# ska-telescope/ska-sdp-screen-fitting

Hardware: AMD Instinct MI355X
Metric: screen-slots/sec (ant×time×freq) + FITS-cube wall-clock, KL 256² screen (higher is better)
Workload: dtype f64

## Files before the change

include/screenfit.h:

```cpp
#ifndef SCREENFIT_H
#define SCREENFIT_H

#include <stddef.h>
#include <stdint.h>

#ifdef __cplusplus
extern "C" {
#endif

#define SF_OK 0
#define SF_EINVAL (-22)
#define SF_ENOMEM (-12)
#define SF_EIO (-5)
#define SF_ENODEV (-19)

#define SF_MAX_DIR 60
#define SF_MAX_FIT_DIR 128
#define SF_MAX_EVAL_DIR 128

#define SF_SCREEN_PHASE 0
#define SF_SCREEN_TEC 1
#define SF_SCREEN_AMPLITUDE 2

#define SF_EVAL_NAN_SCRUB 1u
// ... 21 lines not shown
int sf_synchronize(sf_ctx* ctx);
int sf_stream_create(sf_ctx* ctx, const int* reserve_cus, int n_reserve,
                     void** hip_stream);
int sf_stream_destroy(sf_ctx* ctx, void* hip_stream);
int sf_device_cus(sf_ctx* ctx, int* n_cu);
#define SF_OPT_FIT_GENERAL 1
#define SF_OPT_EVAL_KERNEL 2
#define SF_OPT_EVAL_MAX_BLOCKS 3
#define SF_OPT_FIT_PACK 4
#define SF_OPT_EVAL_KS_PAD 5
#define SF_OPT_EVAL_SLEEP 6
#define SF_OPT_EVAL_XCD_MAP 7
#define SF_OPT_EVAL_GROUPS 8
#define SF_OPT_EVAL_BANDS 9
#define SF_OPT_FIT_LEAN 10
#define SF_OPT_TESS_SLOTS 11
#define SF_OPT_TESS_WAVES 12
#define SF_OPT_TESS_TILE 13
#define SF_OPT_TESS_BOX 14
#define SF_OPT_EVAL_INT 15
#define SF_OPT_EVAL_WG_WAVES 16
#define SF_OPT_FIT_EIG_WAVES 17
#define SF_OPT_FIT_SUBSET_DELETION 18
#define SF_EVAL_KERNEL_AUTO 0
#define SF_EVAL_KERNEL_TILE 1
#define SF_EVAL_KERNEL_LDS4 2
#define SF_EVAL_KERNEL_LDS8 3
#define SF_EVAL_KERNEL_LDS16 4
#define SF_EVAL_KERNEL_LDS8H 5
#define SF_EVAL_KERNEL_LDS16H 6
#define SF_EVAL_KERNEL_TILE3 7
#define SF_EVAL_KERNEL_SHB 8
#define SF_EVAL_KERNEL_WIDE 9
int sf_get_eval_kernel(sf_ctx* ctx, int gain, unsigned flags, int* kernel);
#define SF_EVAL_CONTRACTION_F64 0
#define SF_EVAL_CONTRACTION_I8_DIGITS 1
int sf_get_eval_contraction(sf_ctx* ctx, int gain, unsigned flags, int* contraction);
int sf_set_option(sf_ctx* ctx, int option, int value);
int sf_alloc(sf_ctx* ctx, size_t bytes, void** dev_ptr);
int sf_free(sf_ctx* ctx, void* dev_ptr);
int sf_copy_h2d(sf_ctx* ctx, void* dst_dev, const void* src_host, size_t bytes);
int sf_copy_d2h(sf_ctx* ctx, void* dst_host, const void* src_dev, size_t bytes);

int sf_set_basis(sf_ctx* ctx, const double* pp_host, int D, double r0,
                 double beta);
int sf_set_basis_wide(sf_ctx* ctx, const double* pp_host, int D, double r0,
                      double beta);
int sf_get_basis(sf_ctx* ctx, double* c_host, double* pinv_c_host,
                 double* u_host, double* eig_host);

int sf_set_piercepoints(sf_ctx* ctx, const double* pp_host, int D, double r0,
                        double beta);

int sf_kl_fit(sf_ctx* ctx, const double* phase, const float* weight, int T,
              int F, int A, const int* station_order_host,
              const sf_fit_params* params, double* coef, double* resid,
              float* w_out, int32_t* order_out);

int sf_get_fit_stats(sf_ctx* ctx, int* n_masks, int* n_general);

int sf_get_fit_pool(sf_ctx* ctx, uint64_t* masks_host, double* entries_host,
                    int max_masks, int* n_masks);

int sf_set_grid(sf_ctx* ctx, const double* x_host, int nx,
                const double* y_host, int ny);

int sf_kl_eval(sf_ctx* ctx, const double* coef, int64_t S, float* out,
               int64_t ring_slots, unsigned flags);

int sf_kl_eval_gain(sf_ctx* ctx, const double* coef_phase,
                    const double* coef_xx, const double* coef_yy, int64_t S,
                    float* out, int64_t ring_slots, unsigned flags);
int sf_kl_eval_sums(sf_ctx* ctx, const double* coef_phase,
                    const double* coef_xx, const double* coef_yy, int64_t S,
                    float* out, int64_t ring, unsigned flags,
                    uint32_t* slot_sums);

int sf_kl_eval_values(sf_ctx* ctx, const double* coef, int64_t S, float* out,
                      int64_t ring_slots, unsigned flags);

#define SF_MAX_POINTS 4096
int sf_set_points(sf_ctx* ctx, const double* xy_host, int P);
// ... 17 lines not shown
```

ska-sdp-screen-fitting_amd/csrc/capi.hip:

```cpp
#include <hip/hip_runtime.h>

#include <cmath>
#include <cstring>
#include <string>
#include <vector>

#include "sf_internal.h"

namespace sf {
static thread_local std::string g_last_error;
void set_error(const std::string& msg) { g_last_error = msg; }
}

using sf::set_error;

namespace {

int check_device(int device) {
  int n = 0;
  hipError_t e = hipGetDeviceCount(&n);
  if (e != hipSuccess || n == 0) {
    set_error("no HIP device available");
    return SF_ENODEV;
  }
// ... 73 lines not shown
  hipFree(ctx->d_c);
  hipFree(ctx->d_pinv);
  hipFree(ctx->d_u);
  hipFree(ctx->d_eig);
  hipFree(ctx->d_wide_ws);
  hipFree(ctx->d_wide_w);
  hipFree(ctx->d_wide_o);
  hipFree(ctx->d_cfrag);
  hipFree(ctx->d_pxy);
  hipFree(ctx->d_pfrag);
  hipFree(ctx->d_cdig);
  hipFree(ctx->d_kdig);
  hipFree(ctx->d_kflag);
  if (ctx->kdig_read) (void)hipEventDestroy(ctx->kdig_read);
  hipFree(ctx->d_skip);
  hipFree(ctx->d_st_order);
  hipFree(ctx->d_keys);
  hipFree(ctx->d_ids);
  hipFree(ctx->d_pool_mask);
  hipFree(ctx->d_pool);
  hipFree(ctx->d_pool_status);
  hipFree(ctx->d_pos);
  hipFree(ctx->d_sigma);
  hipFree(ctx->d_class);
  hipFree(ctx->d_counters);
  hipFree(ctx->d_scratch);
  hipFree(ctx->d_wscratch);
  hipFree(ctx->d_oscratch);
  hipFree(ctx->d_gw);
  hipFree(ctx->d_smooth);
  hipFree(ctx->d_tess_tab);
  hipFree(ctx->d_trash);
  delete ctx;
  return SF_OK;
}

int sf_set_stream(sf_ctx* ctx, void* stream) {
  SF_REQUIRE(ctx, SF_EINVAL, "sf_set_stream: NULL context");
  ctx->stream = reinterpret_cast<hipStream_t>(stream);
  return SF_OK;
}

int sf_device_cus(sf_ctx* ctx, int* n_cu) {
  SF_REQUIRE(ctx && n_cu, SF_EINVAL, "sf_device_cus: NULL argument");
  SF_HIP(hipDeviceGetAttribute(n_cu, hipDeviceAttributeMultiprocessorCount,
                               ctx->device));
// ... 28 lines not shown
int sf_stream_destroy(sf_ctx* ctx, void* stream) {
  SF_REQUIRE(ctx && stream, SF_EINVAL, "sf_stream_destroy: bad argument");
  SF_HIP(hipSetDevice(ctx->device));
  SF_HIP(hipStreamDestroy(reinterpret_cast<hipStream_t>(stream)));
  return SF_OK;
}

int sf_set_option(sf_ctx* ctx, int option, int value) {
  SF_REQUIRE(ctx, SF_EINVAL, "sf_set_option: NULL context");
  switch (option) {
    case SF_OPT_FIT_GENERAL:
      ctx->force_general = value != 0;
      return SF_OK;
    case SF_OPT_EVAL_KERNEL:
      SF_REQUIRE(value >= SF_EVAL_KERNEL_AUTO && value <= SF_EVAL_KERNEL_WIDE,
                 SF_EINVAL, "sf_set_option: unknown evaluation kernel");
      ctx->eval_kernel = value;
      return SF_OK;
    case SF_OPT_FIT_PACK:
      ctx->fit_pack = value != 0;
      return SF_OK;
    case SF_OPT_FIT_LEAN:
      ctx->fit_lean = value != 0;
      return SF_OK;
    case SF_OPT_EVAL_KS_PAD:
      SF_REQUIRE(value >= 0 && value <= 3, SF_EINVAL,
                 "sf_set_option: k-step padding must be 0..3");
      ctx->eval_ks_pad = value;
      return SF_OK;
    case SF_OPT_EVAL_SLEEP:
      SF_REQUIRE(value >= 0 && value <= 1000, SF_EINVAL,
                 "sf_set_option: eval sleep must be 0..1000");
      ctx->eval_sleep = value;
      return SF_OK;
    case SF_OPT_EVAL_XCD_MAP:
      SF_REQUIRE(value >= -1 && value <= 1, SF_EINVAL,
                 "sf_set_option: XCD map must be -1, 0 or 1");
      ctx->eval_xcd_map = value;
      return SF_OK;
    case SF_OPT_EVAL_GROUPS:
      SF_REQUIRE(value >= 0 && value <= 256 && (value & (value - 1)) == 0,
                 SF_EINVAL, "sf_set_option: groups must be 0 or a power of two <= 256");
      ctx->eval_groups = value;
      return SF_OK;
    case SF_OPT_EVAL_BANDS:
      SF_REQUIRE(value >= 0 && value <= 128 && (value & (value - 1)) == 0,
// ... 251 lines not shown
  }
  if (ctx->st_order_cap < (size_t)A) {
    SF_TRY(dev_alloc(&ctx->d_st_order, (size_t)A));
    ctx->st_order_cap = (size_t)A;
  }
  SF_HIP(hipMemcpyAsync(ctx->d_st_order, st_order, sizeof(int) * A,
                        hipMemcpyHostToDevice, ctx->stream));
  return sf::launch_fit(ctx, phase, weight, T, F, A, p, coef, resid, w_out,
                        order_out);
}

int sf_get_fit_stats(sf_ctx* ctx, int* n_masks, int* n_general) {
  SF_REQUIRE(ctx, SF_EINVAL, "sf_get_fit_stats: NULL context");
  int c[4] = {0, 0, 0, 0};
  SF_HIP(hipSetDevice(ctx->device));
  SF_HIP(hipStreamSynchronize(ctx->stream));
  if (ctx->d_counters)
    SF_HIP(hipMemcpy(c, ctx->d_counters, sizeof(c), hipMemcpyDeviceToHost));
  if (n_masks) *n_masks = c[0];
  if (n_general) *n_general = c[2];
  return SF_OK;
}

int sf_get_fit_pool(sf_ctx* ctx, uint64_t* masks_host, double* entries_host,
                    int max_masks, int* n_masks) {
  SF_REQUIRE(ctx && n_masks && max_masks >= 0, SF_EINVAL, "sf_get_fit_pool: bad argument");
  SF_REQUIRE(max_masks == 0 || (masks_host && entries_host), SF_EINVAL,
             "sf_get_fit_pool: NULL output");
  SF_REQUIRE(!ctx->wide, SF_EINVAL,
             "sf_get_fit_pool: no mask pool above SF_MAX_DIR directions "
             "(sf_set_basis_wide: every flagged slot decomposes its own subset)");
  SF_HIP(hipSetDevice(ctx->device));
  SF_HIP(hipStreamSynchronize(ctx->stream));
  int c0 = 0;
  if (ctx->d_counters)
    SF_HIP(hipMemcpy(&c0, ctx->d_counters, sizeof(int), hipMemcpyDeviceToHost));
  const int n = ctx->pool_D == ctx->D && (size_t)c0 <= ctx->pool_cap ? c0 : 0;
  *n_masks = n;
  const int k = n < max_masks ? n : max_masks;
  if (k > 0) {
    const size_t entry = (size_t)ctx->D * ctx->D + ctx->D;
    SF_HIP(hipMemcpy(masks_host, ctx->d_pool_mask, k * sizeof(uint64_t),
                     hipMemcpyDeviceToHost));
    SF_HIP(hipMemcpy(entries_host, ctx->d_pool, k * entry * sizeof(double),
                     hipMemcpyDeviceToHost));
  }
// ... 289 lines not shown
```

ska-sdp-screen-fitting_amd/csrc/kl_fit_fast.hip:

```cpp
#include <hip/hip_runtime.h>

#include <algorithm>
#include <cmath>
#include <cstdlib>

#include "sf_internal.h"
#include "sf_wave.h"

namespace sf {

constexpr double kAtol = 1e-3;
constexpr size_t kLdsBytes = 160 * 1024;
constexpr double kTinyW = 1e-3 * 1.001;
constexpr unsigned long long kEmptyKey = 0ull;

__host__ __device__ inline int ldo(int n) { return n | 1; }

__device__ __forceinline__ unsigned long long mix64(unsigned long long x) {
  x ^= x >> 30;
  x *= 0xbf58476d1ce4e5b9ull;
  x ^= x >> 27;
  x *= 0x94d049bb133111ebull;
  x ^= x >> 31;
  return x;
}

__device__ int table_insert(unsigned long long* keys, int cap,
                            unsigned long long key) {
  int h = (int)(mix64(key) & (unsigned long long)(cap - 1));
  for (int probe = 0; probe < cap; ++probe) {
    unsigned long long prev = keys[h];
    if (prev == kEmptyKey) prev = atomicCAS(keys + h, kEmptyKey, key);
    if (prev == kEmptyKey || prev == key) return h;
    h = (h + 1) & (cap - 1);
  }
  return -3;
}
// ... 476 lines not shown
  return (size_t)((c_global ? 1 : 2) * D * ldo(D) + 64) * sizeof(double);
}
__host__ __device__ inline size_t fast_wave_bytes(int D, bool slow, bool lean = false) {
  if (lean) return (size_t)6 * 64 * sizeof(double);
  return (size_t)((slow ? 3 : 2) * D * ldo(D) + 64 + 6 * 64) * sizeof(double) +
         (slow ? 64 * sizeof(double2) + 96 * sizeof(int2) : 0);
}

struct Basis {
  int n;
  bool full;
  int ld;
  const double* U;
  const double* lam;
};

__device__ __noinline__ void nl_sincos(double x, double* s, double* c) { sincos(x, s, c); }
__device__ __noinline__ double nl_atan2(double y, double x) { return atan2(y, x); }
__device__ __noinline__ double nl_log10(double x) { return log10(x); }
__device__ __noinline__ double nl_pow(double x, double y) { return pow(x, y); }
__device__ __noinline__ double nl_log(double x) { return log(x); }
__device__ __noinline__ double nl_fmod(double x, double y) { return fmod(x, y); }

template <bool NI>
struct FitMath {
  static __device__ __forceinline__ void sin_cos(double x, double* s, double* c) {
    if constexpr (NI) nl_sincos(x, s, c); else sincos(x, s, c);
  }
  static __device__ __forceinline__ double arctan2(double y, double x) {
    if constexpr (NI) return nl_atan2(y, x); else return atan2(y, x);
  }
  static __device__ __forceinline__ double lg10(double x) {
    if constexpr (NI) return nl_log10(x); else return log10(x);
  }
  static __device__ __forceinline__ double power(double x, double y) {
    if constexpr (NI) return nl_pow(x, y); else return pow(x, y);
  }
  static __device__ __forceinline__ double ln(double x) {
    if constexpr (NI) return nl_log(x); else return log(x);
  }
  static __device__ __forceinline__ double mod(double x, double y) {
    if constexpr (NI) return nl_fmod(x, y); else return fmod(x, y);
  }
};

template <bool NI = false>
// ... 185 lines not shown
    v0[l] = fabs(lm) > kAtol ? sh / lm : 0.0;
  }
  lds_sync();
  double wa = 0.0;
  if (l < D)
#pragma unroll kMatVecUnroll
    for (int r = 0; r < D; ++r) wa += L.U[l * ld + r] * v0[r];
  lds_sync();
  white_d = wa;
  resid_d = phi_d - model_value<NI>(screen_type, sall);
}

template <bool NI = false>
__device__ __forceinline__ double screen_diff(int screen_type, double val,
                                              double resid) {
  if (screen_type == SF_SCREEN_AMPLITUDE)
    return FitMath<NI>::lg10(val) - FitMath<NI>::lg10(fabs(val - resid));
  return resid;
}

#ifndef SF_FIT_MINW
#define SF_FIT_MINW 4
#endif
template <bool SLOW, int SPW, bool LEAN>
__global__ __launch_bounds__(256, SLOW ? 1 : SF_FIT_MINW) void kl_fit_pass_kernel(
    int it, int niter, int64_t S, int F, int A, int D,
    const double* __restrict__ phase, const double* __restrict__ refph,
    int ref_sub, const double* __restrict__ g_u, const double* __restrict__ g_c,
    const double* __restrict__ g_eig, const int* __restrict__ st_order,
    const uint8_t* __restrict__ cls, int* __restrict__ pos,
    const int* __restrict__ ids, unsigned long long* __restrict__ keys, int cap,
    const double* __restrict__ pool, int pool_cap, int* __restrict__ counters,
    int screen_type, double nsigma, int adjust_order, double* __restrict__ coef,
    double* __restrict__ resid, float* __restrict__ w_out,
    int32_t* __restrict__ order_out) {
#pragma clang fp contract(off)
  extern __shared__ double smem[];
  const int ld = ldo(D);
  using G = Group<SPW>;
  using M = FitMath<!SLOW>;
  constexpr bool NI = !SLOW;
  constexpr bool CG = SPW == 1;
  const int nwaves = blockDim.x / 64;
  const int nslots = nwaves * SPW;
  const int wv = (threadIdx.x / 64) * SPW + G::index();
  const int d = G::lane();
  double* sU = smem;
  double* sC = CG ? nullptr : sU + D * ld;
  double* sl = sU + (CG ? 1 : 2) * D * ld;
  for (int e = threadIdx.x; e < D * D; e += blockDim.x) {
    const int r = e / D, c = e % D;
    sU[r * ld + c] = g_u[e];
    if (!CG) sC[r * ld + c] = g_c[e];
  }
  for (int e = threadIdx.x; e < 64; e += blockDim.x) sl[e] = e < D ? g_eig[e] : 0.0;
  __syncthreads();
  FastLds L;
  L.U = sU;
  L.C = CG ? g_c : sC;
  L.cld = CG ? D : ld;
  L.lam = sl;
  double* wb = sl + 64 + (size_t)wv * (fast_wave_bytes(D, SLOW, LEAN) / sizeof(double));
  if (LEAN) {
    L.Vs = L.G = L.M = L.lams = nullptr;
    L.vec = wb;
    L.cs = nullptr;
    L.pr = nullptr;
  } else {
    L.Vs = wb;
    L.G = wb + D * ld;
    L.M = L.G + D * ld;
    L.lams = (SLOW ? L.M + D * ld : L.G + D * ld);
    L.vec = L.lams + 64;
    L.cs = reinterpret_cast<double2*>(L.vec + 6 * 64);
    L.pr = reinterpret_cast<int2*>(L.cs + 64);
  }
  const uint8_t want = SLOW ? 2 : 0;

  for (int64_t s = (int64_t)blockIdx.x * nslots + wv; s < S;
       s += (int64_t)gridDim.x * nslots) {
    if (SLOW && cls[s] != want) continue;
    const uint8_t cl = SLOW ? want : cls[s];
    const int a = (int)(s % A);
    const int p0 = pos[s];
    const int64_t base = s * D;
    double phi_d = 0.0, w_d = 0.0, white_d = 0.0, resid_d = 0.0;
    if (d < D) {
      phi_d = phase_ref(phase, refph, ref_sub, s, a, A, D, d);
      w_d = (double)w_out[base + d];
      white_d = it == 0 ? 0.0 : coef[base + d];
      resid_d = it == 0 ? 0.0 : resid[base + d];
    }
    double order = (double)order_out[s];
    const double station_order = (double)st_order[a];
    if (cl != want) continue;
    int id = -1;
    if (p0 >= 0) {
      id = ids[p0];
      if (id < 0 || id >= pool_cap) {
        if (d == 0) atomicOr(counters + 3, 1);
        continue;
      }
    } else if (p0 == -3) {
      if (d == 0) atomicOr(counters + 3, 2);
      continue;
// ... 20 lines not shown
          if (d < n_unfl) L.Vs[r * ld + d] = e[r * D + d];
        if (d < n_unfl) L.lams[d] = e[D * D + d];
        lds_sync();
        B.U = L.Vs;
        B.lam = L.lams;
      }
    }
    double phi_p = 0.0, w_p = 0.0;
    {
      double* v4 = L.vec + 256;
      double* v5 = L.vec + 320;
      if (unfl) {
        const int p = G::rank(um);
        v4[p] = phi_d;
        v5[p] = w_d;
      }
      lds_sync();
      if (d < n_unfl) {
        phi_p = v4[d];
        w_p = v5[d];
      }
      lds_sync();
    }
    const double wmax = G::max(unfl ? w_d : -INFINITY);
    const double wmin = -G::max(unfl ? -w_d : -INFINITY);
    const bool uniform = (wmax == wmin);
    if (LEAN && n_unfl > 0 && !uniform) {
      if (d == 0) atomicOr(counters + 3, 4);
      continue;
    }

    if (n_unfl > 0) {
      if (order > n_unfl - 1) order = n_unfl - 1;
      if (it == 0) {
        fit_once<SLOW, SPW, LEAN>(L, B, D, ld, (int)order, screen_type, uniform, wmin,
                       phi_p, w_p, phi_d, w_d, white_d, resid_d);
      } else if (adjust_order) {
        bool hit_upper = false, hit_lower = false, hit_upper2 = false,
             hit_lower2 = false;
        double sign = 1.0, prev_redchi2 = 0.0;
        for (int oi = 0; oi < 4; ++oi) {
          if (oi > 0)
            fit_once<SLOW, SPW, LEAN>(L, B, D, ld, (int)order, screen_type, uniform, wmin,
                           phi_p, w_p, phi_d, w_d, white_d, resid_d);
          if (hit_lower2 || hit_upper2) break;
          double redchi2;
          if (screen_type == SF_SCREEN_PHASE) {
            double sn = 0.0, cn = 0.0;
            if (unfl) M::sin_cos(resid_d, &sn, &cn);
// ... 16 lines not shown
          }
          prev_redchi2 = redchi2;
          const double order_factor = M::power((double)n_unfl - order, 0.2);
          double target = order - sign * order_factor * (1.0 - redchi2);
          target = fmax(station_order, target);
          target = fmin(rint(target), (double)(n_unfl - 1));
          if (target <= 0.0) target = fmin(station_order, (double)(n_unfl - 1));
          if (target == order) break;
          if (target == n_unfl - 1) {
            if (hit_upper) hit_upper2 = true;
            hit_upper = true;
          }
          if (target == station_order) {
            if (hit_lower) hit_lower2 = true;
            hit_lower = true;
          }
          order = target;
        }
      }
    }
    if (it + 1 < niter && screen_type == SF_SCREEN_PHASE) {
      const bool live = d < D;
      if (G::any(live && w_d > 0.0)) {
        double r = M::mod(resid_d, 2.0 * M_PI);
        if (r < -M_PI) r += 2.0 * M_PI;
        if (r > M_PI) r -= 2.0 * M_PI;
        const bool inc = live && (w_d != 0.0) && !isnan(r);
        double sn = 0.0, cn = 0.0;
        if (inc) M::sin_cos(r, &sn, &cn);
        const double cnt = G::sum(inc ? 1.0 : 0.0);
        const double ms = G::sum(sn) / cnt;
        const double mc = G::sum(cn) / cnt;
        const double stdv = sqrt(-2.0 * M::ln(hypot(ms, mc)));
        const bool outl = live && (fabs(r) > nsigma * stdv);
        if (outl) w_d = 0.0;
        if (G::any(outl)) {
          const unsigned long long nm = G::ballot(live && w_d > 0.0);
          if (d == 0) pos[s] = (nm == 0ull) ? -2 : table_insert(keys, cap, nm);
        }
      }
    }
    if (d < D) {
      coef[base + d] = white_d;
      resid[base + d] = resid_d;
      w_out[base + d] = (float)w_d;
    }
    if (d == 0) order_out[s] = (int32_t)order;
  }
}

__global__ __launch_bounds__(256) void kl_block_sigma_kernel(
    int T, int F, int A, int D, const double* __restrict__ phase,
    const double* __restrict__ refph, int ref_sub,
    const uint8_t* __restrict__ skip, int ref_skip, int screen_type,
    const double* __restrict__ resid, const float* __restrict__ w_out,
    double* __restrict__ sigma) {
  __shared__ double red[2][256];
  const int blk = blockIdx.x;
  const int f = blk / A, a = blk % A;
  double sw = 0.0, swr = 0.0;
  if (!(skip[blk] || a == ref_skip)) {
    for (int e = threadIdx.x; e < T * D; e += blockDim.x) {
      const int t = e / D, d = e % D;
      const int64_t s = ((int64_t)t * F + f) * A + a;
      const double w = (double)w_out[s * D + d];
      if (w > 0.0) {
        const double v = phase_ref(phase, refph, ref_sub, s, a, A, D, d);
        const double sd = screen_diff(screen_type, v, resid[s * D + d]);
        swr += w * (sd * sd);
        sw += w;
      }
// ... 145 lines not shown
    const int blocks = n_new < 8192 ? n_new : 8192;
    const int nw = ctx->fit_eig_waves > 0 ? ctx->fit_eig_waves : kEigWavesDefault;
#define SF_LAUNCH_EIG(NW)                                                              \
  do {                                                                                 \
    if (shm > 64 * 1024)                                                               \
      SF_HIP(hipFuncSetAttribute(reinterpret_cast<const void*>(&kl_subset_eig_kernel<NW>), \
                                 hipFuncAttributeMaxDynamicSharedMemorySize, (int)shm)); \
    hipLaunchKernelGGL(kl_subset_eig_kernel<NW>, dim3(blocks), dim3(64 * NW), shm,     \
                       ctx->stream, ctx->d_c, D, ctx->d_pool_mask, (int)ctx->pool_cap, \
                       ctx->d_counters, ctx->d_pool, done);                            \
  } while (0)
    switch (nw) {
      case 1: SF_LAUNCH_EIG(1); break;
      case 2: SF_LAUNCH_EIG(2); break;
      case 4: SF_LAUNCH_EIG(4); break;
      default: SF_LAUNCH_EIG(3); break;
    }
#undef SF_LAUNCH_EIG
    SF_HIP(hipGetLastError());
  }
  return SF_OK;
}

template <bool SLOW, int SPW, bool LEAN>
static int launch_pass_spw(sf_ctx* ctx, int it, const sf_fit_params* p,
                           const RefSpec& r, int64_t S, int F, int A,
                           const double* phase, double* coef, double* resid,
                           float* w_out, int32_t* order_out) {
  const int D = ctx->D;
  const size_t shared = fast_shared_bytes(D, SPW == 1);
  const size_t slot = fast_wave_bytes(D, SLOW, LEAN);
  int nw = 1, best = 0;
  for (int k = 1; k <= 4; ++k) {
    const size_t per_wg = shared + (size_t)k * SPW * slot;
    if (per_wg > kLdsBytes) break;
    const int waves = k * (int)(kLdsBytes / per_wg);
    if (waves > best) {
      best = waves;
      nw = k;
    }
  }
  const size_t shm = shared + (size_t)nw * SPW * slot;
  if (shm > 64 * 1024)
    SF_HIP(hipFuncSetAttribute(
        reinterpret_cast<const void*>(&kl_fit_pass_kernel<SLOW, SPW, LEAN>),
        hipFuncAttributeMaxDynamicSharedMemorySize, (int)shm));
  int64_t blocks = (S + nw * SPW - 1) / (nw * SPW);
  if (blocks > 16384) blocks = 16384;
  hipLaunchKernelGGL((kl_fit_pass_kernel<SLOW, SPW, LEAN>), dim3((unsigned)blocks),
                     dim3(64 * nw), shm, ctx->stream, it, p->niter, S, F, A, D,
                     phase, r.refph, r.sub, ctx->d_u, ctx->d_c, ctx->d_eig,
                     ctx->d_st_order, ctx->d_class, ctx->d_pos, ctx->d_ids,
                     ctx->d_keys, (int)ctx->table_cap, ctx->d_pool,
                     (int)ctx->pool_cap, ctx->d_counters, p->screen_type,
                     p->nsigma, p->adjust_order, coef, resid, w_out, order_out);
  SF_HIP(hipGetLastError());
  return SF_OK;
}

template <bool SLOW>
static int launch_pass(sf_ctx* ctx, int it, const sf_fit_params* p,
                       const RefSpec& r, int64_t S, int F, int A,
                       const double* phase, double* coef, double* resid,
                       float* w_out, int32_t* order_out, bool lean) {
  const bool pack = !SLOW && ctx->D <= 32 && ctx->fit_pack;
  if (!SLOW && lean && ctx->fit_lean) {
    if (pack)
      return launch_pass_spw<false, 2, true>(ctx, it, p, r, S, F, A, phase, coef,
                                             resid, w_out, order_out);
    return launch_pass_spw<false, 1, true>(ctx, it, p, r, S, F, A, phase, coef,
                                           resid, w_out, order_out);
  }
  if (pack)
    return launch_pass_spw<SLOW, 2, false>(ctx, it, p, r, S, F, A, phase, coef,
                                           resid, w_out, order_out);
  return launch_pass_spw<SLOW, 1, false>(ctx, it, p, r, S, F, A, phase, coef, resid,
                                         w_out, order_out);
}

int launch_block_sigma(sf_ctx* ctx, int T, int F, int A, const double* phase,
                       const RefSpec& r, int screen_type, const double* resid,
                       const float* w_out) {
  hipLaunchKernelGGL(kl_block_sigma_kernel, dim3(F * A), dim3(256), 0,
                     ctx->stream, T, F, A, ctx->D, phase, r.refph, r.sub,
                     ctx->d_skip, r.skip, screen_type, resid, w_out,
                     ctx->d_sigma);
  SF_HIP(hipGetLastError());
  return SF_OK;
}
// ... 47 lines not shown
  if (ctx->sigma_cap < (size_t)F * A) {
    size_t c = 0;
    if (ctx->d_sigma) (void)hipFree(ctx->d_sigma);
    ctx->d_sigma = nullptr;
    SF_TRYF(grow(&ctx->d_sigma, c, (size_t)F * A));
    ctx->sigma_cap = (size_t)F * A;
  }
  const size_t tcap = next_pow2((size_t)(2 * p->niter + 2) * (size_t)S + 64);
  if (ctx->table_cap < tcap) {
    size_t c1 = 0, c2 = 0;
    if (ctx->d_keys) (void)hipFree(ctx->d_keys);
    if (ctx->d_ids) (void)hipFree(ctx->d_ids);
    ctx->d_keys = nullptr;
    ctx->d_ids = nullptr;
    SF_TRYF(grow(&ctx->d_keys, c1, tcap));
    SF_TRYF(grow(&ctx->d_ids, c2, tcap));
    ctx->table_cap = tcap;
  }
  if (!ctx->d_counters) {
    size_t c = 0;
    SF_TRYF(grow(&ctx->d_counters, c, 8));
  }
  SF_TRYF(ensure_pool(ctx, 1024));
  const int cap = (int)ctx->table_cap;
  SF_HIP(hipMemsetAsync(ctx->d_keys, 0, ctx->table_cap * sizeof(unsigned long long),
                        ctx->stream));
  SF_HIP(hipMemsetAsync(ctx->d_ids, 0xff, ctx->table_cap * sizeof(int), ctx->stream));
  SF_HIP(hipMemsetAsync(ctx->d_counters, 0, 8 * sizeof(int), ctx->stream));

  {
    const int gw = D <= 8 ? 8 : D <= 16 ? 16 : D <= 32 ? 32 : 64;
    const int64_t per_block = 4 * (64 / gw);
    const dim3 grid((unsigned)((S + per_block - 1) / per_block));
#define SF_CLASSIFY(W)                                                          \
  hipLaunchKernelGGL(kl_classify_kernel<W>, grid, dim3(256), 0, ctx->stream,    \
                     weight, S, F, A, D, ctx->d_st_order, ctx->d_skip, r.skip,  \
                     ctx->d_keys, cap, ctx->d_pos, ctx->d_class,               \
                     ctx->d_counters, coef, resid, w_out, order_out)
    switch (gw) {
      case 8: SF_CLASSIFY(8); break;
      case 16: SF_CLASSIFY(16); break;
      case 32: SF_CLASSIFY(32); break;
      default: SF_CLASSIFY(64); break;
    }
#undef SF_CLASSIFY
    SF_HIP(hipGetLastError());
// ... 38 lines not shown
```

ska-sdp-screen-fitting_amd/csrc/sf_internal.h:

```cpp
#pragma once

#include <hip/hip_runtime.h>

#include <cstdint>
#include <string>

#include "screenfit.h"

namespace sf {

void set_error(const std::string& msg);

#define SF_HIP(call)                                                        \
  do {                                                                      \
    hipError_t e_ = (call);                                                 \
    if (e_ != hipSuccess) {                                                 \
      ::sf::set_error(std::string(#call) + ": " + hipGetErrorString(e_));   \
      return SF_EIO;                                                        \
    }                                                                       \
  } while (0)

#define SF_REQUIRE(cond, code, msg) \
  do {                              \
    if (!(cond)) {                  \
// ... 75 lines not shown
  int pt_tiles = 0;
  int pt_ks_pad = 0;
  int pt_cus = 0;
  double* d_pxy = nullptr;
  double* d_pfrag = nullptr;
  uint8_t* d_skip = nullptr;
  size_t skip_cap = 0;
  int* d_st_order = nullptr;
  size_t st_order_cap = 0;
  unsigned long long* d_keys = nullptr;
  int* d_ids = nullptr;
  size_t table_cap = 0;
  unsigned long long* d_pool_mask = nullptr;
  double* d_pool = nullptr;
  int fit_eig_waves = 0;
  int fit_subset_deletion = 1;
  size_t pool_cap = 0;
  uint8_t* d_pool_status = nullptr;
  size_t pool_status_cap = 0;
  int pool_D = 0;
  int* d_pos = nullptr;
  uint8_t* d_class = nullptr;
  double* d_sigma = nullptr;
  size_t sigma_cap = 0;
  size_t slot_cap = 0;
  int* d_counters = nullptr;
  double* d_scratch = nullptr;
  size_t scratch_cap = 0;
  float* d_wscratch = nullptr;
  int32_t* d_oscratch = nullptr;
  double* d_gw = nullptr;
  size_t gw_cap = 0;
  double gw_sigma = -1.0;
  float* d_trash = nullptr;
  float* d_smooth = nullptr;
  size_t smooth_cap = 0;
  float* d_tess_tab = nullptr;
  size_t tess_tab_cap = 0;
  int force_general = 0;
  int eval_kernel = SF_EVAL_KERNEL_AUTO;
  int64_t eval_max_blocks = 0;
  int eval_ks_pad = 0;
  int eval_sleep = 0;
  int eval_xcd_map = -1;
  int eval_groups = 0;
  int eval_bands = 0;
  int tess_slots = 0;
  int tess_waves = 0;
  int tess_tile = 0;
  int tess_box = -1;
  int fit_pack = 1;
  int fit_lean = 1;
};

namespace sf {
constexpr int kEvalMaxKS = 15;
constexpr int kEvalWideMaxKS = SF_MAX_EVAL_DIR / 4;
inline bool eval_int_applies(const sf_ctx* ctx, bool gain, unsigned flags,
                             bool out_aligned16) {
  return !gain && ctx->dig_ok && ctx->d_cdig && ctx->eval_int != 0 &&
         (flags & SF_EVAL_FAST_SINCOS) && ctx->n_pix % 4 == 0 && out_aligned16 &&
         ctx->ksteps >= 12 && ctx->ksteps <= kEvalMaxKS;
}

struct RefSpec {
  int sub = -1;
  const double* refph = nullptr;
  int skip = -1;
};
RefSpec ref_spec(const sf_fit_params* p, int A);
int launch_skip(sf_ctx* ctx, const double* phase, const float* weight, int T,
                int F, int A, const RefSpec& r);
int launch_fit_general(sf_ctx* ctx, const int* slot_list, const int* n_list,
                       int64_t max_slots, const double* phase,
                       const float* weight, int T, int F, int A,
// ... 45 lines not shown
```

ska-sdp-screen-fitting_amd/ska_sdp_screen_fitting_amd/_lib.py:

```python

import contextlib
import ctypes
import os
import threading

import numpy as np

_HERE = os.path.dirname(os.path.abspath(__file__))
LIB_PATH = os.environ.get("SCREENFIT_LIB", os.path.join(_HERE, "libscreenfit.so"))

SF_SCREEN_PHASE = 0
SF_SCREEN_TEC = 1
SF_SCREEN_AMPLITUDE = 2
SF_EVAL_NAN_SCRUB = 1
SF_EVAL_FAST_SINCOS = 1 << 8
SF_EVAL_NT_STORES = 1 << 9
SF_EVAL_BIG_ENDIAN = 1 << 10
SF_MAX_DIR = 60
SF_MAX_FIT_DIR = 128
SF_MAX_EVAL_DIR = 128
SF_MAX_POINTS = 4096
SF_OPT_FIT_GENERAL = 1
SF_OPT_EVAL_KERNEL = 2
SF_OPT_EVAL_MAX_BLOCKS = 3
SF_OPT_FIT_PACK = 4
SF_OPT_EVAL_KS_PAD = 5
SF_OPT_EVAL_SLEEP = 6
SF_OPT_EVAL_XCD_MAP = 7
SF_OPT_EVAL_GROUPS = 8
SF_OPT_EVAL_BANDS = 9
SF_OPT_FIT_LEAN = 10
SF_OPT_TESS_SLOTS = 11
SF_OPT_TESS_WAVES = 12
SF_OPT_TESS_TILE = 13
SF_OPT_TESS_BOX = 14
SF_OPT_EVAL_INT = 15
SF_OPT_EVAL_WG_WAVES = 16
SF_OPT_FIT_EIG_WAVES = 17
SF_OPT_FIT_SUBSET_DELETION = 18
SF_EVAL_KERNEL_AUTO = 0
SF_EVAL_KERNEL_TILE = 1
SF_EVAL_KERNEL_LDS4 = 2
SF_EVAL_KERNEL_LDS8 = 3
SF_EVAL_KERNEL_LDS16 = 4
SF_EVAL_KERNEL_LDS8H = 5
SF_EVAL_KERNEL_LDS16H = 6
SF_EVAL_KERNEL_TILE3 = 7
SF_EVAL_KERNEL_SHB = 8
SF_EVAL_KERNEL_WIDE = 9
EVAL_KERNEL_NAMES = {SF_EVAL_KERNEL_TILE: "kl_eval_kernel",
                     SF_EVAL_KERNEL_LDS4: "kl_eval_lds_kernel<4 waves>",
                     SF_EVAL_KERNEL_LDS8: "kl_eval_lds_kernel<8 waves>",
                     SF_EVAL_KERNEL_LDS16: "kl_eval_lds_kernel<16 waves>",
                     SF_EVAL_KERNEL_LDS8H: "kl_eval_lds_kernel<8 waves, 2 tiles>",
                     SF_EVAL_KERNEL_LDS16H: "kl_eval_lds_kernel<16 waves, 2 tiles>",
                     SF_EVAL_KERNEL_TILE3: "kl_eval_kernel<3 waves/SIMD>",
                     SF_EVAL_KERNEL_SHB: "kl_eval_kernel<Cpix in LDS>",
                     SF_EVAL_KERNEL_WIDE: "kl_eval_wide_kernel"}

EXPORTED = (
    "sf_version", "sf_last_error", "sf_create", "sf_destroy", "sf_set_stream",
    "sf_synchronize", "sf_set_option", "sf_get_eval_kernel", "sf_get_eval_contraction", "sf_alloc", "sf_free", "sf_copy_h2d", "sf_copy_d2h",
    "sf_set_basis", "sf_set_basis_wide", "sf_set_piercepoints", "sf_get_basis", "sf_kl_fit", "sf_get_fit_stats", "sf_get_fit_pool",
    "sf_stream_create", "sf_stream_destroy", "sf_device_cus",
    "sf_set_grid", "sf_kl_eval", "sf_kl_eval_gain", "sf_kl_eval_sums",
    "sf_tess_fill", "sf_smooth",
    "sf_set_points", "sf_kl_eval_points", "sf_kl_eval_point_values",
    "sf_kl_eval_values",
)


_identity = {}


def library_identity(path=None):
    import hashlib
    p = os.path.realpath(path or LIB_PATH)
    if p not in _identity:
        h = hashlib.sha256()
        with open(p, "rb") as fh:
            for blk in iter(lambda: fh.read(1 << 20), b""):
                h.update(blk)
        _identity[p] = {"sha16": h.hexdigest()[:16], "bytes": os.path.getsize(p)}
    return dict(_identity[p])


# ... 28 lines not shown
                                ctypes.c_int, ctypes.c_double)
        i64 = ctypes.c_int64
        sig = {
            "sf_version": ([], ctypes.c_char_p),
            "sf_last_error": ([], ctypes.c_char_p),
            "sf_create": ([c_int, ctypes.POINTER(vp)], c_int),
            "sf_destroy": ([vp], c_int),
            "sf_set_stream": ([vp, vp], c_int),
            "sf_synchronize": ([vp], c_int),
            "sf_set_option": ([vp, c_int, c_int], c_int),
            "sf_get_eval_kernel": ([vp, c_int, ctypes.c_uint, ip], c_int),
            "sf_get_eval_contraction": ([vp, c_int, ctypes.c_uint, ip], c_int),
            "sf_alloc": ([vp, ctypes.c_size_t, ctypes.POINTER(vp)], c_int),
            "sf_free": ([vp, vp], c_int),
            "sf_copy_h2d": ([vp, vp, vp, ctypes.c_size_t], c_int),
            "sf_copy_d2h": ([vp, vp, vp, ctypes.c_size_t], c_int),
            "sf_set_basis": ([vp, vp, c_int, c_dbl, c_dbl], c_int),
            "sf_set_basis_wide": ([vp, vp, c_int, c_dbl, c_dbl], c_int),
            "sf_set_piercepoints": ([vp, vp, c_int, c_dbl, c_dbl], c_int),
            "sf_get_basis": ([vp, vp, vp, vp, vp], c_int),
            "sf_kl_fit": ([vp, vp, vp, c_int, c_int, c_int, ip,
                           ctypes.POINTER(FitParams), vp, vp, vp, vp], c_int),
            "sf_get_fit_stats": ([vp, ip, ip], c_int),
            "sf_get_fit_pool": ([vp, vp, vp, c_int, ip], c_int),
            "sf_set_grid": ([vp, vp, c_int, vp, c_int], c_int),
            "sf_kl_eval": ([vp, vp, i64, vp, i64, ctypes.c_uint], c_int),
            "sf_stream_create": ([vp, ctypes.POINTER(c_int), c_int,
                                  ctypes.POINTER(vp)], c_int),
            "sf_stream_destroy": ([vp, vp], c_int),
            "sf_device_cus": ([vp, ctypes.POINTER(c_int)], c_int),
            "sf_kl_eval_gain": ([vp, vp, vp, vp, i64, vp, i64, ctypes.c_uint],
                                c_int),
            "sf_kl_eval_sums": ([vp, vp, vp, vp, i64, vp, i64, ctypes.c_uint, vp],
                                c_int),
            "sf_tess_fill": ([vp, vp, c_int, c_int, vp, vp, vp, c_int, i64, vp,
                              i64, c_dbl, ctypes.c_uint], c_int),
            "sf_smooth": ([vp, vp, c_int, c_int, i64, c_dbl, ctypes.c_uint], c_int),
            "sf_set_points": ([vp, vp, c_int], c_int),
            "sf_kl_eval_points": ([vp, vp, vp, vp, i64, vp, ctypes.c_uint], c_int),
            "sf_kl_eval_point_values": ([vp, vp, i64, vp], c_int),
            "sf_kl_eval_values": ([vp, vp, i64, vp, i64, ctypes.c_uint], c_int),
        }
        for name, (args, res) in sig.items():
            fn = getattr(lib, name)
            fn.argtypes = args
            fn.restype = res
# ... 132 lines not shown
            ref_phase=None):
        so = np.ascontiguousarray(station_order, dtype=np.int32)
        if so.shape != (A,):
            raise ValueError(f"station_order: shape {so.shape}, expected ({A},)")
        n = int(T) * int(F) * int(A) * self.D
        prm = FitParams(int(screen_type), int(niter), float(nsigma),
                        int(bool(adjust_order)), int(ref_ant), int(ant_offset),
                        self._dev(ref_phase, np.float64, int(T) * int(F) * self.D,
                             "ref_phase"))
        _check(self.lib.sf_kl_fit(
            self.h, self._dev(phase, np.float64, n, "phase"),
            self._dev(weight, np.float32, n, "weight"), int(T), int(F), int(A),
            so.ctypes.data_as(ctypes.POINTER(ctypes.c_int)),
            ctypes.byref(prm), self._dev(coef, np.float64, n, "coef"),
            self._dev(resid, np.float64, n, "resid"),
            self._dev(w_out, np.float32, n, "w_out"),
            self._dev(order_out, np.int32, n // max(self.D, 1), "order_out")),
            "sf_kl_fit")

    def fit_stats(self):
        nm, ng = ctypes.c_int(), ctypes.c_int()
        _check(self.lib.sf_get_fit_stats(self.h, ctypes.byref(nm), ctypes.byref(ng)),
               "sf_get_fit_stats")
        return {"n_masks": nm.value, "n_general": ng.value}

    def fit_pool(self):
        n = ctypes.c_int(0)
        _check(self.lib.sf_get_fit_pool(self.h, None, None, 0, ctypes.byref(n)),
               "sf_get_fit_pool")
        D = self.D
        masks = np.zeros(n.value, np.uint64)
        ent = np.zeros((n.value, D * D + D))
        if n.value:
            _check(self.lib.sf_get_fit_pool(self.h, masks.ctypes.data, ent.ctypes.data,
                                            n.value, ctypes.byref(n)), "sf_get_fit_pool")
        order = np.argsort(masks, kind="stable")
        masks, ent = masks[order], ent[order]
        for k, m in enumerate(masks):
            n = bin(int(m)).count("1")
            u = ent[k, :D * D].reshape(D, D)
            u[n:, :] = 0.0
            u[:, n:] = 0.0
            ent[k, D * D + n:] = 0.0
        return masks, ent

    def set_grid(self, x, y):
        x = np.ascontiguousarray(x, dtype=np.float64)
# ... 151 lines not shown
```

Baseline: 6.290 million.

## Retire converged fit slots early and skip them in later iterations

Adds an early-finish variant of the lean packed phase fit pass. A slot is marked finished when it flags no outliers and its order adjustment is stable, and later iterations skip it. The variant also replaces the min/max reductions with a broadcast-and-any check, skips fmod when residuals are already in range, and reads pow(k,0.2) from a precomputed table. This cuts repeated per-iteration work on converged slots, at the risk of diverging from the reference if the stability test misses a later change.

```diff
diff --git a/include/screenfit.h b/include/screenfit.h
--- a/include/screenfit.h
+++ b/include/screenfit.h
@@ -67,6 +67,7 @@
 #define SF_OPT_EVAL_WG_WAVES 16
 #define SF_OPT_FIT_EIG_WAVES 17
 #define SF_OPT_FIT_SUBSET_DELETION 18
+#define SF_OPT_FIT_EARLY_FINISH 19
 #define SF_EVAL_KERNEL_AUTO 0
 #define SF_EVAL_KERNEL_TILE 1
 #define SF_EVAL_KERNEL_LDS4 2
@@ -103,6 +104,7 @@
               float* w_out, int32_t* order_out);
 
 int sf_get_fit_stats(sf_ctx* ctx, int* n_masks, int* n_general);
+int sf_get_fit_path_stats(sf_ctx* ctx, int* n_early);
 
 int sf_get_fit_pool(sf_ctx* ctx, uint64_t* masks_host, double* entries_host,
                     int max_masks, int* n_masks);
diff --git a/ska-sdp-screen-fitting_amd/csrc/capi.hip b/ska-sdp-screen-fitting_amd/csrc/capi.hip
--- a/ska-sdp-screen-fitting_amd/csrc/capi.hip
+++ b/ska-sdp-screen-fitting_amd/csrc/capi.hip
@@ -119,6 +119,7 @@
   hipFree(ctx->d_pool_status);
   hipFree(ctx->d_pos);
   hipFree(ctx->d_sigma);
+  hipFree(ctx->d_fit_pow);
   hipFree(ctx->d_class);
   hipFree(ctx->d_counters);
   hipFree(ctx->d_scratch);
@@ -193,6 +194,9 @@
       return SF_OK;
     case SF_OPT_FIT_LEAN:
       ctx->fit_lean = value != 0;
+      return SF_OK;
+    case SF_OPT_FIT_EARLY_FINISH:
+      ctx->fit_early_finish = value != 0;
       return SF_OK;
     case SF_OPT_EVAL_KS_PAD:
       SF_REQUIRE(value >= 0 && value <= 3, SF_EINVAL,
@@ -490,6 +494,17 @@
   return SF_OK;
 }
 
+int sf_get_fit_path_stats(sf_ctx* ctx, int* n_early) {
+  SF_REQUIRE(ctx, SF_EINVAL, "sf_get_fit_path_stats: NULL context");
+  int c = 0;
+  SF_HIP(hipSetDevice(ctx->device));
+  SF_HIP(hipStreamSynchronize(ctx->stream));
+  if (ctx->d_counters && !ctx->wide)
+    SF_HIP(hipMemcpy(&c, ctx->d_counters + 6, sizeof(int), hipMemcpyDeviceToHost));
+  if (n_early) *n_early = c;
+  return SF_OK;
+}
+
 int sf_get_fit_pool(sf_ctx* ctx, uint64_t* masks_host, double* entries_host,
                     int max_masks, int* n_masks) {
   SF_REQUIRE(ctx && n_masks && max_masks >= 0, SF_EINVAL, "sf_get_fit_pool: bad argument");
diff --git a/ska-sdp-screen-fitting_amd/csrc/kl_fit_fast.hip b/ska-sdp-screen-fitting_amd/csrc/kl_fit_fast.hip
--- a/ska-sdp-screen-fitting_amd/csrc/kl_fit_fast.hip
+++ b/ska-sdp-screen-fitting_amd/csrc/kl_fit_fast.hip
@@ -3,6 +3,7 @@
 #include <algorithm>
 #include <cmath>
 #include <cstdlib>
+#include <type_traits>
 
 #include "sf_internal.h"
 #include "sf_wave.h"
@@ -13,6 +14,7 @@
 constexpr size_t kLdsBytes = 160 * 1024;
 constexpr double kTinyW = 1e-3 * 1.001;
 constexpr unsigned long long kEmptyKey = 0ull;
+constexpr uint8_t kClassFinished = 3;
 
 __host__ __device__ inline int ldo(int n) { return n | 1; }
 
@@ -535,6 +537,10 @@
 __device__ __noinline__ double nl_log(double x) { return log(x); }
 __device__ __noinline__ double nl_fmod(double x, double y) { return fmod(x, y); }
 
+__global__ __launch_bounds__(64) void kl_pow_table_kernel(double* __restrict__ tab) {
+  if (threadIdx.x < 32) tab[threadIdx.x] = nl_pow((double)threadIdx.x, 0.2);
+}
+
 template <bool NI>
 struct FitMath {
   static __device__ __forceinline__ void sin_cos(double x, double* s, double* c) {
@@ -766,16 +772,18 @@
 #ifndef SF_FIT_MINW
 #define SF_FIT_MINW 4
 #endif
-template <bool SLOW, int SPW, bool LEAN>
+template <bool SLOW, int SPW, bool LEAN, bool EARLY = false>
 __global__ __launch_bounds__(256, SLOW ? 1 : SF_FIT_MINW) void kl_fit_pass_kernel(
     int it, int niter, int64_t S, int F, int A, int D,
     const double* __restrict__ phase, const double* __restrict__ refph,
     int ref_sub, const double* __restrict__ g_u, const double* __restrict__ g_c,
     const double* __restrict__ g_eig, const int* __restrict__ st_order,
-    const uint8_t* __restrict__ cls, int* __restrict__ pos,
+    std::conditional_t<EARLY, uint8_t*, const uint8_t*> __restrict__ cls,
+    int* __restrict__ pos,
     const int* __restrict__ ids, unsigned long long* __restrict__ keys, int cap,
     const double* __restrict__ pool, int pool_cap, int* __restrict__ counters,
-    int screen_type, double nsigma, int adjust_order, double* __restrict__ coef,
+    int screen_type, double nsigma, int adjust_order,
+    const double* __restrict__ pow_tab, double* __restrict__ coef,
     double* __restrict__ resid, float* __restrict__ w_out,
     int32_t* __restrict__ order_out) {
 #pragma clang fp contract(off)
@@ -785,6 +793,8 @@
   using M = FitMath<!SLOW>;
   constexpr bool NI = !SLOW;
   constexpr bool CG = SPW == 1;
+  static_assert(!EARLY || (!SLOW && SPW == 2 && LEAN), "early finish: two-slot lean pass");
+  constexpr bool early = EARLY;
   const int nwaves = blockDim.x / 64;
   const int nslots = nwaves * SPW;
   const int wv = (threadIdx.x / 64) * SPW + G::index();
@@ -798,6 +808,9 @@
     if (!CG) sC[r * ld + c] = g_c[e];
   }
   for (int e = threadIdx.x; e < 64; e += blockDim.x) sl[e] = e < D ? g_eig[e] : 0.0;
+  if constexpr (EARLY) {
+    if (threadIdx.x >= 32 && threadIdx.x < 64) sl[threadIdx.x] = pow_tab[threadIdx.x - 32];
+  }
   __syncthreads();
   FastLds L;
   L.U = sU;
@@ -820,11 +833,13 @@
     L.pr = reinterpret_cast<int2*>(L.cs + 64);
   }
   const uint8_t want = SLOW ? 2 : 0;
+  int n_early = 0;
 
   for (int64_t s = (int64_t)blockIdx.x * nslots + wv; s < S;
        s += (int64_t)gridDim.x * nslots) {
     if (SLOW && cls[s] != want) continue;
     const uint8_t cl = SLOW ? want : cls[s];
+    if (early && it > 0 && cl != want) continue;
     const int a = (int)(s % A);
     const int p0 = pos[s];
     const int64_t base = s * D;
@@ -891,9 +906,16 @@
       }
       lds_sync();
     }
-    const double wmax = G::max(unfl ? w_d : -INFINITY);
-    const double wmin = -G::max(unfl ? -w_d : -INFINITY);
-    const bool uniform = (wmax == wmin);
+    double wmin;
+    bool uniform;
+    if constexpr (EARLY) {
+      wmin = G::bcast(w_d, um ? __builtin_ctzll(um) : 0);
+      uniform = !G::any(unfl && w_d != wmin);
+    } else {
+      const double wmax = G::max(unfl ? w_d : -INFINITY);
+      wmin = -G::max(unfl ? -w_d : -INFINITY);
+      uniform = (wmax == wmin);
+    }
     if (LEAN && n_unfl > 0 && !uniform) {
       if (d == 0) atomicOr(counters + 3, 4);
       continue;
@@ -956,21 +978,55 @@
     if (it + 1 < niter && screen_type == SF_SCREEN_PHASE) {
       const bool live = d < D;
       if (G::any(live && w_d > 0.0)) {
-        double r = M::mod(resid_d, 2.0 * M_PI);
+        double r = resid_d;
+        if (!early || __ballot(!(fabs(resid_d) < 2.0 * M_PI)) != 0ull)
+          r = M::mod(resid_d, 2.0 * M_PI);
         if (r < -M_PI) r += 2.0 * M_PI;
         if (r > M_PI) r -= 2.0 * M_PI;
         const bool inc = live && (w_d != 0.0) && !isnan(r);
         double sn = 0.0, cn = 0.0;
         if (inc) M::sin_cos(r, &sn, &cn);
-        const double cnt = G::sum(inc ? 1.0 : 0.0);
+        const double cnt = EARLY ? (double)__popcll(G::ballot(inc)) : G::sum(inc ? 1.0 : 0.0);
         const double ms = G::sum(sn) / cnt;
         const double mc = G::sum(cn) / cnt;
         const double stdv = sqrt(-2.0 * M::ln(hypot(ms, mc)));
         const bool outl = live && (fabs(r) > nsigma * stdv);
         if (outl) w_d = 0.0;
-        if (G::any(outl)) {
+        const bool flagged = G::any(outl);
+        if (flagged) {
           const unsigned long long nm = G::ballot(live && w_d > 0.0);
           if (d == 0) pos[s] = (nm == 0ull) ? -2 : table_insert(keys, cap, nm);
+        } else if constexpr (EARLY) {
+          bool stable = true;
+          if (adjust_order) {
+            double s2 = unfl ? sn : 0.0, c2 = unfl ? cn : 0.0;
+            const bool same = inc && __double_as_longlong(r) == __double_as_longlong(resid_d);
+            if (__ballot(unfl && !same) != 0ull) {
+              s2 = c2 = 0.0;
+              if (unfl) M::sin_cos(resid_d, &s2, &c2);
+            }
+            const double ww = unfl ? w_d : 0.0;
+            const double sw = (double)n_unfl * wmin;
+            const double m1 = G::sum(s2 * s2 * ww) / sw;
+            const double m2 = G::sum(c2 * c2 * ww) / sw;
+            const double redchi2 = (1.0 - hypot(m1, m2)) * sw / (n_unfl - order);
+            const double k = (double)n_unfl - order;
+            const int ki = (int)k;
+            double order_factor;
+            if (ki >= 0 && ki < 32 && (double)ki == k)
+              order_factor = sl[32 + ki];
+            else
+              order_factor = M::power(k, 0.2);
+            double target = order - order_factor * (1.0 - redchi2);
+            target = fmax(station_order, target);
+            target = fmin(rint(target), (double)(n_unfl - 1));
+            if (target <= 0.0) target = fmin(station_order, (double)(n_unfl - 1));
+            stable = target == order;
+          }
+          if (stable && d == 0) {
+            cls[s] = kClassFinished;
+            ++n_early;
+          }
         }
       }
     }
@@ -981,6 +1037,7 @@
     }
     if (d == 0) order_out[s] = (int32_t)order;
   }
+  if (n_early > 0) atomicAdd(counters + 6, n_early);
 }
 
 __global__ __launch_bounds__(256) void kl_block_sigma_kernel(
@@ -1172,7 +1229,7 @@
   return SF_OK;
 }
 
-template <bool SLOW, int SPW, bool LEAN>
+template <bool SLOW, int SPW, bool LEAN, bool EARLY = false>
 static int launch_pass_spw(sf_ctx* ctx, int it, const sf_fit_params* p,
                            const RefSpec& r, int64_t S, int F, int A,
                            const double* phase, double* coef, double* resid,
@@ -1193,17 +1250,18 @@
   const size_t shm = shared + (size_t)nw * SPW * slot;
   if (shm > 64 * 1024)
     SF_HIP(hipFuncSetAttribute(
-        reinterpret_cast<const void*>(&kl_fit_pass_kernel<SLOW, SPW, LEAN>),
+        reinterpret_cast<const void*>(&kl_fit_pass_kernel<SLOW, SPW, LEAN, EARLY>),
         hipFuncAttributeMaxDynamicSharedMemorySize, (int)shm));
   int64_t blocks = (S + nw * SPW - 1) / (nw * SPW);
   if (blocks > 16384) blocks = 16384;
-  hipLaunchKernelGGL((kl_fit_pass_kernel<SLOW, SPW, LEAN>), dim3((unsigned)blocks),
+  hipLaunchKernelGGL((kl_fit_pass_kernel<SLOW, SPW, LEAN, EARLY>), dim3((unsigned)blocks),
                      dim3(64 * nw), shm, ctx->stream, it, p->niter, S, F, A, D,
                      phase, r.refph, r.sub, ctx->d_u, ctx->d_c, ctx->d_eig,
                      ctx->d_st_order, ctx->d_class, ctx->d_pos, ctx->d_ids,
                      ctx->d_keys, (int)ctx->table_cap, ctx->d_pool,
                      (int)ctx->pool_cap, ctx->d_counters, p->screen_type,
-                     p->nsigma, p->adjust_order, coef, resid, w_out, order_out);
+                     p->nsigma, p->adjust_order, ctx->d_fit_pow, coef, resid, w_out,
+                     order_out);
   SF_HIP(hipGetLastError());
   return SF_OK;
 }
@@ -1215,6 +1273,9 @@
                        float* w_out, int32_t* order_out, bool lean) {
   const bool pack = !SLOW && ctx->D <= 32 && ctx->fit_pack;
   if (!SLOW && lean && ctx->fit_lean) {
+    if (pack && ctx->fit_early_finish && p->screen_type == SF_SCREEN_PHASE)
+      return launch_pass_spw<false, 2, true, true>(ctx, it, p, r, S, F, A, phase, coef,
+                                                   resid, w_out, order_out);
     if (pack)
       return launch_pass_spw<false, 2, true>(ctx, it, p, r, S, F, A, phase, coef,
                                              resid, w_out, order_out);
@@ -1308,6 +1369,13 @@
     SF_TRYF(grow(&ctx->d_counters, c, 8));
   }
   SF_TRYF(ensure_pool(ctx, 1024));
+  if (!ctx->d_fit_pow) {
+    size_t c = 0;
+    SF_TRYF(grow(&ctx->d_fit_pow, c, 32));
+    hipLaunchKernelGGL(kl_pow_table_kernel, dim3(1), dim3(64), 0, ctx->stream,
+                       ctx->d_fit_pow);
+    SF_HIP(hipGetLastError());
+  }
   const int cap = (int)ctx->table_cap;
   SF_HIP(hipMemsetAsync(ctx->d_keys, 0, ctx->table_cap * sizeof(unsigned long long),
                         ctx->stream));
diff --git a/ska-sdp-screen-fitting_amd/csrc/sf_internal.h b/ska-sdp-screen-fitting_amd/csrc/sf_internal.h
--- a/ska-sdp-screen-fitting_amd/csrc/sf_internal.h
+++ b/ska-sdp-screen-fitting_amd/csrc/sf_internal.h
@@ -121,6 +121,7 @@
   int* d_pos = nullptr;
   uint8_t* d_class = nullptr;
   double* d_sigma = nullptr;
+  double* d_fit_pow = nullptr;
   size_t sigma_cap = 0;
   size_t slot_cap = 0;
   int* d_counters = nullptr;
@@ -150,6 +151,7 @@
   int tess_box = -1;
   int fit_pack = 1;
   int fit_lean = 1;
+  int fit_early_finish = 1;
 };
 
 namespace sf {
diff --git a/ska-sdp-screen-fitting_amd/ska_sdp_screen_fitting_amd/_lib.py b/ska-sdp-screen-fitting_amd/ska_sdp_screen_fitting_amd/_lib.py
--- a/ska-sdp-screen-fitting_amd/ska_sdp_screen_fitting_amd/_lib.py
+++ b/ska-sdp-screen-fitting_amd/ska_sdp_screen_fitting_amd/_lib.py
@@ -38,6 +38,7 @@
 SF_OPT_EVAL_WG_WAVES = 16
 SF_OPT_FIT_EIG_WAVES = 17
 SF_OPT_FIT_SUBSET_DELETION = 18
+SF_OPT_FIT_EARLY_FINISH = 19
 SF_EVAL_KERNEL_AUTO = 0
 SF_EVAL_KERNEL_TILE = 1
 SF_EVAL_KERNEL_LDS4 = 2
@@ -61,7 +62,7 @@
 EXPORTED = (
     "sf_version", "sf_last_error", "sf_create", "sf_destroy", "sf_set_stream",
     "sf_synchronize", "sf_set_option", "sf_get_eval_kernel", "sf_get_eval_contraction", "sf_alloc", "sf_free", "sf_copy_h2d", "sf_copy_d2h",
-    "sf_set_basis", "sf_set_basis_wide", "sf_set_piercepoints", "sf_get_basis", "sf_kl_fit", "sf_get_fit_stats", "sf_get_fit_pool",
+    "sf_set_basis", "sf_set_basis_wide", "sf_set_piercepoints", "sf_get_basis", "sf_kl_fit", "sf_get_fit_stats", "sf_get_fit_path_stats", "sf_get_fit_pool",
     "sf_stream_create", "sf_stream_destroy", "sf_device_cus",
     "sf_set_grid", "sf_kl_eval", "sf_kl_eval_gain", "sf_kl_eval_sums",
     "sf_tess_fill", "sf_smooth",
@@ -136,6 +137,7 @@
             "sf_kl_fit": ([vp, vp, vp, c_int, c_int, c_int, ip,
                            ctypes.POINTER(FitParams), vp, vp, vp, vp], c_int),
             "sf_get_fit_stats": ([vp, ip, ip], c_int),
+            "sf_get_fit_path_stats": ([vp, ip], c_int),
             "sf_get_fit_pool": ([vp, vp, vp, c_int, ip], c_int),
             "sf_set_grid": ([vp, vp, c_int, vp, c_int], c_int),
             "sf_kl_eval": ([vp, vp, i64, vp, i64, ctypes.c_uint], c_int),
@@ -314,7 +316,10 @@
         nm, ng = ctypes.c_int(), ctypes.c_int()
         _check(self.lib.sf_get_fit_stats(self.h, ctypes.byref(nm), ctypes.byref(ng)),
                "sf_get_fit_stats")
-        return {"n_masks": nm.value, "n_general": ng.value}
+        ne = ctypes.c_int()
+        _check(self.lib.sf_get_fit_path_stats(self.h, ctypes.byref(ne)),
+               "sf_get_fit_path_stats")
+        return {"n_masks": nm.value, "n_general": ng.value, "n_early": ne.value}
 
     def fit_pool(self):
         n = ctypes.c_int(0)
```

Result: no change. 6.318 million (median of 6 runs) (+0.4%).
